# MatthewRalston/kmerdb

Measured on AMD Instinct MI355X. Metric: k-mers counted/sec at k=12, synthetic 150 bp FASTQ, higher is better.
Workload: dtype u64

## Files before the change

### include/kdbhip.h

```cpp
#ifndef KDBHIP_H
#define KDBHIP_H

#include <stddef.h>
#include <stdint.h>

#ifdef __cplusplus
extern "C" {
#endif

#define KDB_ABI_VERSION 6

#define KDB_OK               0
#define KDB_ERR_ARG          1
#define KDB_ERR_HIP          2
#define KDB_ERR_SHORT_READ   3
#define KDB_ERR_BAD_RESIDUE  4
#define KDB_ERR_NOMEM        5
#define KDB_ERR_STATE        6

#define KDB_N_DROP    0
#define KDB_N_EXPAND  1

typedef struct kdb_engine kdb_engine;

// ... 14 lines not shown
#define KDB_SUBMIT_PINNED     1
#define KDB_SUBMIT_CONTINUES  2
int kdb_submit_ex(kdb_engine *e, const uint8_t *bases, size_t nbytes,
                  const uint64_t *read_offsets, size_t nreads, int flags);
int kdb_host_alloc(void **out, size_t nbytes);
int kdb_host_free(void *p);

int kdb_submit_device(kdb_engine *e, void *d_bases, size_t nbytes,
                      const void *d_read_offsets, size_t nreads);

int kdb_submit_device_const(kdb_engine *e, const void *d_bases, size_t nbytes,
                            const void *d_read_offsets, size_t nreads);

int kdb_sync(kdb_engine *e);

int kdb_finish(kdb_engine *e, uint64_t *counts_out, uint64_t *total_kmers, uint64_t *unique_kmers);

int kdb_table_stats(kdb_engine *e, uint64_t *counts_out, uint64_t *sum_out, uint64_t *unique_out);

int kdb_nullomers(kdb_engine *e, int folded, uint64_t *ids_out, uint64_t cap, uint64_t *n_out);

#define KDB_REDUCE_MAX 16
int kdb_reduce(kdb_engine *const *engines, int n, int root);

#define KDB_GRAM_MAX 64
#define KDB_GRAM_BLOCK 4
#define KDB_GRAM_WG_BINS 512
int kdb_gram(int device_id, const void *const *d_vectors, int n, uint64_t nbins,
             uint64_t *sums_out   ,
             uint64_t *gram_out   ,
             double   *kernel_ms_out );

int kdb_fold_file(kdb_engine *e, uint64_t *total_kmers, uint64_t *unique_kmers);
int kdb_fold_file_into(kdb_engine *e, kdb_engine *acc, uint64_t *total_kmers, uint64_t *unique_kmers);
int kdb_finish_folded(kdb_engine *e, uint64_t *counts_out, uint64_t *total_kmers, uint64_t *unique_kmers);

int kdb_table(kdb_engine *e, void **d_table_out, uint64_t *nbins_out);

int kdb_error_counts(kdb_engine *e, uint64_t *n_short_reads, uint64_t *n_bad_residues);

int kdb_create_ids(int k, int canonicalize, int device_id, kdb_engine **out);

int kdb_shred(kdb_engine *e, const uint8_t *seq, size_t nbytes,
              uint64_t *ids_out, uint64_t *pos_out, size_t cap, size_t *n_out);

int kdb_window_ids(kdb_engine *e, const uint8_t *bases, size_t nbytes,
// ... 23 lines not shown
int kdb_gz_read(kdb_gz *g, uint8_t *dst, size_t cap, size_t *n_out);
int kdb_gz_close(kdb_gz *g);

int kdb_write_kdb_rows(const char *path, const uint64_t *counts, uint64_t nbins, uint64_t total_kmers,
                       int compresslevel, int nthreads, uint64_t *nblocks_out);
#define KDB_ENCODER_DEFAULT (-1)
#define KDB_ENCODER_ROWS      0
#define KDB_ENCODER_ZLIB      1
int kdb_write_kdb_rows_ex(const char *path, const uint64_t *counts, uint64_t nbins, uint64_t total_kmers,
                          int compresslevel, int nthreads, int encoder, uint64_t *nblocks_out);
int kdb_format_frequency(uint64_t count, uint64_t total, char *buf, size_t cap);
int kdb_copy_back_and_write_kdb_rows(kdb_engine *e, int folded, uint64_t *counts_out, const char *path, uint64_t total_kmers,
                                     int compresslevel, int nthreads, int encoder, uint64_t *nblocks_out);
int kdb_read_kdb_rows(const char *path, uint64_t nbins, uint64_t *kmer_ids_out, uint64_t *counts_out, double *frequencies_out,
                      int nthreads, uint64_t *nrows_out);

#define KDB_KERNEL_MARK          0
#define KDB_KERNEL_COUNT         1
#define KDB_KERNEL_SCATTER       2
#define KDB_KERNEL_SCATTER_L2    3
#define KDB_KERNEL_PAGE_SORT     4
#define KDB_KERNEL_PAGE_HIST     5
#define KDB_KERNEL_STATS         6
#define KDB_N_KERNELS            7
int         kdb_prof_enable(kdb_engine *e, int on);
int         kdb_prof_reset(kdb_engine *e);
int         kdb_prof_get(kdb_engine *e, int kernel_id, double *total_ms, uint64_t *launches);
const char *kdb_prof_kernel_name(int kernel_id);

int         kdb_hbm_pattern_count(void);
const char *kdb_hbm_pattern_name(int i);
int         kdb_hbm_pattern_probe(int device_id, double *gb_per_s_out, int n_out);
int kdb_set_option(kdb_engine *e, const char *name, int64_t value);
int kdb_get_option(kdb_engine *e, const char *name, int64_t *value);

#ifdef __cplusplus
}
#endif
#endif
```

### kmerdb_amd/_abi.py

```python
import ctypes
import os
import subprocess

_HERE = os.path.dirname(os.path.abspath(__file__))
LIB_PATH = os.environ.get("KDB_LIB") or os.path.join(_HERE, "libkdbhip.so")
CSRC = os.path.join(_HERE, "csrc")
INCLUDE = os.path.join(os.path.dirname(_HERE), "include")

KDB_OK, KDB_ERR_ARG, KDB_ERR_HIP, KDB_ERR_SHORT_READ, KDB_ERR_BAD_RESIDUE, KDB_ERR_NOMEM, KDB_ERR_STATE = range(7)
KDB_N_DROP, KDB_N_EXPAND = 0, 1
KDB_SUBMIT_PINNED, KDB_SUBMIT_CONTINUES = 1, 2
KDB_N_KERNELS = 7
KDB_GRAM_MAX, KDB_GRAM_BLOCK, KDB_GRAM_WG_BINS = 64, 4, 512
ABI_VERSION = 6

_u8p = ctypes.POINTER(ctypes.c_uint8)
_u64p = ctypes.POINTER(ctypes.c_uint64)
_vp = ctypes.c_void_p
SYMBOLS = (
    ("kdb_abi_version", ctypes.c_int, []),
    ("kdb_last_error", ctypes.c_char_p, []),
    ("kdb_device_count", ctypes.c_int, [ctypes.POINTER(ctypes.c_int)]),
    ("kdb_create", ctypes.c_int, [ctypes.c_int, ctypes.c_int, ctypes.c_int, ctypes.c_int, _vp, ctypes.POINTER(_vp)]),
    ("kdb_destroy", ctypes.c_int, [_vp]),
    ("kdb_reset", ctypes.c_int, [_vp]),
    ("kdb_submit", ctypes.c_int, [_vp, _vp, ctypes.c_size_t, _vp, ctypes.c_size_t]),
    ("kdb_submit_pinned", ctypes.c_int, [_vp, _vp, ctypes.c_size_t, _vp, ctypes.c_size_t]),
    ("kdb_submit_ex", ctypes.c_int, [_vp, _vp, ctypes.c_size_t, _vp, ctypes.c_size_t, ctypes.c_int]),
    ("kdb_host_alloc", ctypes.c_int, [ctypes.POINTER(_vp), ctypes.c_size_t]),
    ("kdb_host_free", ctypes.c_int, [_vp]),
    ("kdb_submit_device", ctypes.c_int, [_vp, _vp, ctypes.c_size_t, _vp, ctypes.c_size_t]),
    ("kdb_submit_device_const", ctypes.c_int, [_vp, _vp, ctypes.c_size_t, _vp, ctypes.c_size_t]),
    ("kdb_sync", ctypes.c_int, [_vp]),
    ("kdb_finish", ctypes.c_int, [_vp, _vp, _u64p, _u64p]),
    ("kdb_table_stats", ctypes.c_int, [_vp, _vp, _u64p, _u64p]),
    ("kdb_nullomers", ctypes.c_int, [_vp, ctypes.c_int, _vp, ctypes.c_uint64, _u64p]),
    ("kdb_reduce", ctypes.c_int, [ctypes.POINTER(ctypes.c_void_p), ctypes.c_int, ctypes.c_int]),
    ("kdb_gram", ctypes.c_int, [ctypes.c_int, ctypes.POINTER(ctypes.c_void_p), ctypes.c_int, ctypes.c_uint64, _u64p, _u64p,
                                ctypes.POINTER(ctypes.c_double)]),
    ("kdb_fold_file", ctypes.c_int, [_vp, _u64p, _u64p]),
    ("kdb_fold_file_into", ctypes.c_int, [_vp, _vp, _u64p, _u64p]),
    ("kdb_finish_folded", ctypes.c_int, [_vp, _vp, _u64p, _u64p]),
    ("kdb_create_ids", ctypes.c_int, [ctypes.c_int, ctypes.c_int, ctypes.c_int, ctypes.POINTER(_vp)]),
    ("kdb_table", ctypes.c_int, [_vp, ctypes.POINTER(_vp), _u64p]),
    ("kdb_error_counts", ctypes.c_int, [_vp, _u64p, _u64p]),
    ("kdb_shred", ctypes.c_int, [_vp, _vp, ctypes.c_size_t, _vp, _vp, ctypes.c_size_t, ctypes.POINTER(ctypes.c_size_t)]),
    ("kdb_window_ids", ctypes.c_int, [_vp, _vp, ctypes.c_size_t, _vp, ctypes.c_size_t, _vp]),
    ("kdb_parse_fastq", ctypes.c_int, [_vp, ctypes.c_size_t, ctypes.c_int, _vp, ctypes.c_size_t, _vp, ctypes.c_size_t, _vp,
                                       ctypes.POINTER(ctypes.c_size_t), ctypes.POINTER(ctypes.c_size_t), ctypes.POINTER(ctypes.c_size_t)]),
    ("kdb_parse_fastq_mt", ctypes.c_int, [_vp, ctypes.c_size_t, ctypes.c_int, _vp, ctypes.c_size_t, _vp, ctypes.c_size_t, _vp,
                                          ctypes.POINTER(ctypes.c_size_t), ctypes.POINTER(ctypes.c_size_t), ctypes.POINTER(ctypes.c_size_t), ctypes.c_int]),
    ("kdb_parse_fasta", ctypes.c_int, [_vp, ctypes.c_size_t, _vp, ctypes.c_size_t, _vp, ctypes.c_size_t, _vp,
                                       ctypes.POINTER(ctypes.c_size_t), ctypes.POINTER(ctypes.c_size_t)]),
    ("kdb_parse_fasta_chunk", ctypes.c_int, [_vp, ctypes.c_size_t, ctypes.c_int, ctypes.c_int, _vp, ctypes.c_size_t, _vp, ctypes.c_size_t, _vp,
                                             ctypes.POINTER(ctypes.c_size_t), ctypes.POINTER(ctypes.c_size_t), ctypes.POINTER(ctypes.c_size_t),
                                             ctypes.POINTER(ctypes.c_int)]),
    ("kdb_bgzf_inflate", ctypes.c_int, [_vp, ctypes.c_size_t, _vp, ctypes.c_size_t, ctypes.c_int, ctypes.POINTER(ctypes.c_size_t),
                                        ctypes.POINTER(ctypes.c_size_t)]),
    ("kdb_bgzf_scan", ctypes.c_int, [ctypes.c_char_p, _vp, _vp, ctypes.c_size_t, ctypes.POINTER(ctypes.c_size_t)]),
    ("kdb_gz_open", ctypes.c_int, [ctypes.c_char_p, ctypes.POINTER(_vp)]),
    ("kdb_gz_read", ctypes.c_int, [_vp, _vp, ctypes.c_size_t, ctypes.POINTER(ctypes.c_size_t)]),
    ("kdb_gz_close", ctypes.c_int, [_vp]),
# ... 100 lines not shown
```

### kmerdb_amd/csrc/kdb_engine.hip

```cpp
#include <hip/hip_runtime.h>

#include <cstdarg>
#include <cstddef>
#include <cstdio>
#include <cstdlib>
#include <algorithm>
#include <atomic>
#include <cstring>
#include <string>
#include <thread>
#include <vector>

#include "../../include/kdbhip.h"
#include "kdb_kernels.hip.h"
#include "kdb_hist.hip.h"
#include "kdb_scatter.hip.h"
#include "kdb_scatter_host.hip.h"
#include "kdb_smallk.hip.h"
#include "kdb_probe.hip.h"
#include "kdb_gram.hip.h"
#include "kdb_hostparse.cpp.h"
#include "kdb_kdbwriter.cpp.h"

namespace {

thread_local std::string g_err;

int fail(int code, const char *fmt, ...)
{
    char buf[1024];
    va_list ap;
    va_start(ap, fmt);
    vsnprintf(buf, sizeof buf, fmt, ap);
    va_end(ap);
    g_err = buf;
    return code;
}

#define HIP_TRY(expr)                                                                         \
    do {                                                                                      \
        hipError_t _e = (expr);                                                               \
        if (_e != hipSuccess)                                                                 \
            return fail(KDB_ERR_HIP, "%s failed: %s (%s:%d)", #expr, hipGetErrorString(_e),   \
                        __FILE__, __LINE__);                                                  \
    } while (0)

constexpr int NBUF = 2;
const char *const KERNEL_NAMES[KDB_N_KERNELS] = {
    "lens+mark_reads_kernel", "count_kernel", "scatter_bases_kernel", "scatter_ids_kernel", "pages_sort_kernels", "page_hist_kernel", "stats_kernel"};

struct ProfSpan { hipEvent_t a, b; int kernel; };

void parallel_copy(uint8_t *dst, const uint8_t *src, size_t n, int nthreads)
{
    const size_t min_piece = 4u << 20;
    int t = (int)std::min<size_t>((size_t)std::max(nthreads, 1), std::max<size_t>(n / min_piece, 1));
    if (t <= 1) { if (n) memcpy(dst, src, n); return; }
    std::vector<std::thread> th;
    th.reserve((size_t)t - 1);
    const size_t piece = (n / (size_t)t + 63) & ~(size_t)63;
    for (int i = 1; i < t; i++) {
        const size_t a = std::min(n, piece * (size_t)i), b = std::min(n, piece * (size_t)(i + 1));
        if (b > a) th.emplace_back([=] { memcpy(dst + a, src + a, b - a); });
    }
    memcpy(dst, src, std::min(n, piece));
    for (auto &x : th) x.join();
}

void touch_pages(void *buf, size_t n, int nthreads)
{
    if (n < (64u << 20)) return;
    uint8_t *p = (uint8_t *)buf;
// ... 43 lines not shown
    hipEvent_t ev_acc_done[2] = {nullptr, nullptr};
    hipEvent_t ev_acc_copied = nullptr;
    hipEvent_t ev_pin[2] = {nullptr, nullptr};
    bool pin_used[2] = {false, false};
    int pin_idx = 0;
    bool acc_inflight[2] = {false, false};
    int acc_slot = 0;
    size_t acc_nb = 0, acc_nr = 0;
    bool acc_ready = false;

    int64_t algo = 0;
    int min_len = 0;
    int smallk_old = 0;
    kdb::PagedOptions opt;
    kdb::ScatterState sc;
    int overlap = 0;
    int overlap_hist_cus = 0;
    int overlap_mask_mode = 0;
    bool compute_masked = false;
    hipStream_t s_hist = nullptr;
    kdb::OverlapState ov;
    kdb::TwoLevelPaged tp;
    int64_t oom_fallbacks = 0;

    bool tableless = false;
    uint8_t *sh_seq = nullptr; size_t sh_seq_cap = 0;
    uint64_t *sh_offs = nullptr; size_t sh_offs_cap = 0;
    unsigned long long *sh_ids = nullptr; size_t sh_ids_cap = 0;
    kdb::DevCounters *sh_ctr = nullptr;

    unsigned long long *d_acc_table = nullptr;
    uint64_t folded_files = 0, folded_total = 0;
    uint64_t d2h_bytes = 0;
    uint64_t bytes_in = 0;

    bool prof = false;
    std::vector<ProfSpan> spans;
    std::vector<hipEvent_t> ev_pool;
    double prof_ms[KDB_N_KERNELS] = {0};
    uint64_t prof_n[KDB_N_KERNELS] = {0};
};

namespace {

struct DeviceGuard {
    int prev = -1;
// ... 126 lines not shown
    HIP_TRY(hipExtStreamCreateWithCUMask(&e->s_compute, (uint32_t)ms.size(), ms.data()));
    e->compute_masked = true;
    HIP_TRY(hipExtStreamCreateWithCUMask(&e->s_hist, (uint32_t)mh.size(), mh.data()));
    e->ov.grid = 2u * (uint32_t)(ncu - given);
    return KDB_OK;
}

enum : int { BATCH_HOST_FED = 1, BATCH_CONST_INPUT = 2 };
int grow(void **p, size_t *cap, size_t need_bytes);
int launch_batch(kdb_engine *e, uint8_t *d_bases, size_t nbytes, const uint64_t *d_offs, size_t nreads, int first_is_continuation, int flags);

int flush_accumulated(kdb_engine *e)
{
    if (!e->acc_ready || e->acc_nr == 0) return KDB_OK;
    const int s = e->acc_slot;
    HIP_TRY(hipEventRecord(e->ev_acc_copied, e->s_copy));
    HIP_TRY(hipStreamWaitEvent(e->s_compute, e->ev_acc_copied, 0));
    int rc = launch_batch(e, e->d_acc_bases[s], e->acc_nb, e->d_acc_offs[s], e->acc_nr, 0, BATCH_HOST_FED);
    if (rc != KDB_OK) return rc;
    HIP_TRY(hipEventRecord(e->ev_acc_done[s], e->s_compute));
    e->acc_inflight[s] = true;
    e->acc_slot = s ^ 1;
    e->acc_nb = e->acc_nr = 0;
    return KDB_OK;
}

int launch_batch(kdb_engine *e, uint8_t *d_bases, size_t nbytes, const uint64_t *d_offs, size_t nreads, int first_is_continuation, int flags)
{
    if (nreads == 0) return KDB_OK;
    if (e->tableless) return fail(KDB_ERR_STATE, "this engine was created by kdb_create_ids: it has no count vector");
    const uint64_t ntiles = (nbytes + kdb::TILE_BYTES - 1) / kdb::TILE_BYTES;
    if (ntiles > 0x7FFFFFFFull) return fail(KDB_ERR_ARG, "batch too large: %zu bytes", nbytes);
    bool marked = false;
    auto mark = [&]() {
        ProfScope ps(e, KDB_KERNEL_MARK);
        const unsigned mg = (unsigned)std::min<uint64_t>((nreads + 255) / 256, 4096);
        if (flags & BATCH_CONST_INPUT)
            hipLaunchKernelGGL(kdb::require_uniform_kernel, dim3(1), dim3(1), 0, e->s_compute, e->d_ctr);
        else {
            hipLaunchKernelGGL(kdb::mark_reads_kernel, dim3(mg), dim3(256), 0, e->s_compute, d_bases, d_offs, (uint64_t)nreads,
                               first_is_continuation, e->d_ctr);
            marked = true;
        }
    };
    auto unmark = [&]() {
        if (!marked) return;
// ... 8 lines not shown
        const size_t need = ((nbytes >> kdb::FIRST_REC_SHIFT) + 2) * sizeof(uint32_t);
        if (e->first_rec_cap < need && e->d_first_rec) HIP_TRY(hipStreamSynchronize(e->s_compute));
        int grc = grow((void **)&e->d_first_rec, &e->first_rec_cap, need);
        if (grc == KDB_ERR_NOMEM) no_first_rec = true;
        else if (grc != KDB_OK) return grc;
    }
    {
        ProfScope ps(e, KDB_KERNEL_MARK);
        const dim3 grid((unsigned)((nreads + 255) / 256)), block(256);
        HIP_TRY(hipMemsetAsync(&e->d_ctr->neg_min_len, 0, kdb::PER_BATCH_WORDS * sizeof(unsigned long long), e->s_compute));
        const dim3 lgrid(grid.x < 1024u ? grid.x : 1024u);
        hipLaunchKernelGGL(kdb::lens_kernel, lgrid, block, 0, e->s_compute, d_offs, (uint64_t)nreads, (uint64_t)nbytes,
                           e->min_len > 0 ? e->min_len : e->k, first_is_continuation, e->d_ctr, e->d_first_rec);
    }
    if (nbytes == 0) return KDB_OK;
    if (nreads > 0xFFFFFFF0ull) return fail(KDB_ERR_ARG, "batch of %zu records: at most 2^32 - 16 per submit", nreads);
    e->bytes_in += nbytes;
    const kdb::RecStarts rs{d_offs, e->d_first_rec, (uint32_t)nreads, first_is_continuation ? 1u : 0u};
    int algo = (int)e->algo;
    if (algo == 0 || algo == 3) algo = 2;
    if (no_first_rec && algo == 2) { algo = 1; e->oom_fallbacks++; e->tp.table_is_zero = false; }
    const bool paged2 = algo == 2 && e->k > e->opt.one_level_max_k;
    if (!paged2 || e->n_mode == KDB_N_EXPAND || !e->opt.defer) e->tp.table_is_zero = false;
    if (algo == 2) {
        EngineProf hook(e);
        const bool ex = e->n_mode == KDB_N_EXPAND;
        const kdb::ScBatch batch{d_bases, nbytes, rs, e->k, e->canonical, ex, e->d_table, e->d_ctr};
        int rc;
        if (e->k <= kdb::SMALLK_LDS_MAX_K && !e->smallk_old)
            rc = kdb::smallk_lds_count(e->s_compute, d_bases, nbytes, rs, e->k, e->canonical, ex, e->opt.grid, e->d_table, e->d_ctr, hook);
        else if (e->k <= kdb::SMALLK_MAX) {
            mark();
            rc = kdb::smallk_count(e->s_compute, d_bases, nbytes, e->k, e->canonical, ex, e->d_table, e->d_ctr, hook);
            unmark();
        }
        else if (e->k <= e->opt.one_level_max_k) {
            rc = 3;
            if (e->overlap && e->s_hist && !ex) rc = kdb::scatter_count_overlapped(e->ov, e->opt, e->s_compute, e->s_hist, batch, hook);
            if (rc == 3) {
                { const int jrc = overlap_join(e); if (jrc != KDB_OK) return jrc; }
                rc = kdb::scatter_count(e->sc, e->opt, e->s_compute, batch, hook);
            }
        }
        else {
            const size_t lost = nreads * (size_t)(e->k - 1);
            rc = kdb::twolevel_paged_count(e->tp, e->opt, e->s_compute, batch, nbytes > lost ? nbytes - lost : 0, hook);
        }
        if (rc == 2) { e->oom_fallbacks++; algo = 1; e->tp.table_is_zero = false; }
        else if (rc != 0) return fail(KDB_ERR_HIP, "LDS-histogram path failed: %s", kdb::partition_error());
    }
    if (algo == 1) {
        { const int jrc = overlap_join(e); if (jrc != KDB_OK) return jrc; }
        mark();
        {
            ProfScope ps(e, KDB_KERNEL_COUNT);
            const bool ex = (e->n_mode == KDB_N_EXPAND);
            const dim3 grid((unsigned)ntiles), block(kdb::TPB);
#define KDB_LAUNCH_DIRECT(ID, EX)                                                                              \
    hipLaunchKernelGGL((kdb::count_direct_kernel<ID, EX>), grid, block, 0, e->s_compute, d_bases, (uint64_t)nbytes, \
                       e->k, e->canonical, e->d_table, e->d_ctr)
            if (e->k <= 16) { if (ex) KDB_LAUNCH_DIRECT(uint32_t, true); else KDB_LAUNCH_DIRECT(uint32_t, false); }
            else            { if (ex) KDB_LAUNCH_DIRECT(uint64_t, true); else KDB_LAUNCH_DIRECT(uint64_t, false); }
#undef KDB_LAUNCH_DIRECT
        }
        unmark();
    }
    if (e->n_mode == KDB_N_EXPAND && e->d_worklist) {
        ProfScope ps(e, KDB_KERNEL_COUNT);
        hipLaunchKernelGGL(kdb::expand_worklist_kernel, dim3(1024), dim3(256), 0, e->s_compute, e->d_table, e->d_ctr, e->k, e->canonical);
    }
    if (e->n_mode == KDB_N_DROP) {
        ProfScope ps(e, KDB_KERNEL_MARK);
        hipLaunchKernelGGL(kdb::resolve_suspects_kernel, dim3(4), dim3(256), 0, e->s_compute, (const uint8_t *)d_bases, (uint64_t)nbytes, d_offs, (uint64_t)nreads,
                           e->k, e->d_ctr);
    }
    HIP_TRY(hipGetLastError());
    return KDB_OK;
}

int flush_pending_paged(kdb_engine *e)
{
    if (e->tp.pending == 0) return KDB_OK;
    EngineProf hook(e);
    if (kdb::twolevel_paged_flush(e->tp, e->opt, e->s_compute, e->d_table, e->d_ctr, hook)) return fail(KDB_ERR_HIP, "LDS-histogram path failed: %s", kdb::partition_error());
    return KDB_OK;
}

int check_errors(kdb_engine *e)
{
    kdb::DevCounters c;
    HIP_TRY(hipMemcpy(&c, e->d_ctr, sizeof c, hipMemcpyDeviceToHost));
    if (c.n_short)
// ... 76 lines not shown
    hipLaunchKernelGGL((kdbprobe::pattern<RM, WM, NR, NW>), dim3(512), dim3(512), 0, st, src, sb, dst, db, steps, sink);
}
using namespace kdbprobe;
#define KDB_PROBE(name, RM, WM, NR, NW) {name, probe_launch<RM, WM, NR, NW>, (uint32_t)(NR * (RM == R_PAGES15 ? 1536 : RM ? 1024 : 0)), (uint32_t)(NW * (WM ? 1024 : 0))}
const ProbePattern PROBES[] = {
    KDB_PROBE("stream_read", R_STREAM, W_NONE, 4, 0),
    KDB_PROBE("stream_write", R_NONE, W_STREAM, 0, 4),
    KDB_PROBE("pages_1k_read", R_PAGES, W_NONE, 4, 0),
    KDB_PROBE("lines_64_write", R_NONE, W_LINES_SC1, 0, 2),
    KDB_PROBE("pieces_128_write", R_NONE, W_CHUNK128_SC1, 0, 2),
    KDB_PROBE("scatter_64", R_STREAM, W_LINES_SC1, 1, 2),
    KDB_PROBE("scatter_128", R_STREAM, W_CHUNK128_SC1, 1, 2),
    KDB_PROBE("level1_64", R_STREAM, W_LINES_SC1, 1, 3),
    KDB_PROBE("level1_128", R_STREAM, W_CHUNK128_SC1, 1, 3),
    KDB_PROBE("level2_64", R_PAGES15, W_LINES_SC1, 2, 2),
    KDB_PROBE("level2_128", R_PAGES15, W_CHUNK128_SC1, 2, 2),
};
#undef KDB_PROBE
constexpr int N_PROBES = (int)(sizeof(PROBES) / sizeof(PROBES[0]));
}

namespace {
enum OptBefore { OPT_NOTHING, OPT_FLUSH_PENDING , OPT_SYNC_AND_STREAMS ,
                 OPT_NO_STAGING  };
struct OptRow {
    const char *name;
    int64_t (*get)(kdb_engine *);
    void (*set)(kdb_engine *, int64_t) = nullptr;
    bool boolean = false;
    int64_t lo = INT64_MIN, hi = INT64_MAX;
    OptBefore before = OPT_NOTHING;
    const char *hint = "";
    int64_t multiple_of = 1;
};
#define KDB_OPT_RO(field) [](kdb_engine *e) { return (int64_t)e->field; }
#define KDB_OPT(field) KDB_OPT_RO(field), [](kdb_engine *e, int64_t v) { e->field = (decltype(e->field))v; }
const OptRow OPTIONS[] = {
    {"algo", KDB_OPT(algo), false, 0, 3, OPT_NOTHING, " (0 auto, 1 direct atomics, 2 LDS-histogram paths)"},
    {"min_len", KDB_OPT(min_len), false, 0, 64},
    {"copy_threads", KDB_OPT(copy_threads), false, 1, 64},
    {"smallk_old", KDB_OPT(smallk_old), true},
    {"accum_bytes", KDB_OPT(accum_bytes), false, -1, INT64_MAX, OPT_NO_STAGING, " (-1 auto, 0 off, else bytes)"},
    {"stage_bytes", KDB_OPT(stage_bytes), false, 4096, INT64_MAX, OPT_NO_STAGING, " (>=4096, multiple of 16)", 16},
    {"stage_reads", KDB_OPT(stage_reads), false, 1, INT64_MAX, OPT_NO_STAGING},
    {"overlap", KDB_OPT(overlap), true, 0, 1024, OPT_SYNC_AND_STREAMS},
    {"overlap_hist_cus", KDB_OPT(overlap_hist_cus), false, 0, 1024, OPT_SYNC_AND_STREAMS},
    {"overlap_mask_mode", KDB_OPT(overlap_mask_mode), false, 0, 1024, OPT_SYNC_AND_STREAMS},
    {"sc_grid", KDB_OPT(opt.grid), false, 0, 1024, OPT_NOTHING, " (0..1024)"},
    {"sc_lo_bits", KDB_OPT(opt.lo_bits), false, 0, kdb::SC_LO_BITS_MAX, OPT_FLUSH_PENDING, " (0 = the default of the path, 1..15)"},
    {"sc_contig_pages", KDB_OPT(opt.contig_pages), true},
    {"sc_wide_lines", KDB_OPT(opt.wide_lines), true},
    {"l1_wide_lines", KDB_OPT(opt.l1_wide), true},
    {"l2_wide_lines", KDB_OPT(opt.l2_wide), true},
    {"l1_one_round", KDB_OPT(opt.l1_one_round), true},
    {"l1_compiled_k", KDB_OPT(opt.l1k), true},
    {"one_level_max_k", KDB_OPT(opt.one_level_max_k), false, 12, kdb::SC1_K, OPT_FLUSH_PENDING, " (12 or 13)"},
    {"defer_flush", KDB_OPT(opt.defer), true},
    {"pending_budget", KDB_OPT(opt.budget_bytes), false, 0, INT64_MAX},
    {"reserve_bytes", KDB_OPT(opt.reserve_bytes), false, 0, INT64_MAX},
    {"arena_grow", KDB_OPT(opt.grow), false, 0, 2, OPT_NOTHING, " (0 never, 1 when it pays, 2 whenever the arena has filled up)"},
    {"arena_batches", KDB_OPT(opt.first_batches), false, 1, kdb::PAGED_PENDING_MAX, OPT_NOTHING, " (1..64: the arena's first size, in batches like the first one)"},
    {"k", KDB_OPT_RO(k)},
    {"arena_budget_bytes", [](kdb_engine *e) { return (int64_t)(e->opt.budget_bytes ? e->opt.budget_bytes : e->tp.budget_decided); }},
    {"free_at_sizing", KDB_OPT_RO(tp.free_at_sizing)},
    {"overlap_scatter_grid", KDB_OPT_RO(ov.grid)},
    {"oom_fallbacks", KDB_OPT_RO(oom_fallbacks)},
    {"pending_batches", KDB_OPT_RO(tp.pending)},
    {"d2h_bytes", KDB_OPT_RO(d2h_bytes)},
    {"folded_files", KDB_OPT_RO(folded_files)},
    {"bytes_in", KDB_OPT_RO(bytes_in)},
// ... 127 lines not shown
        if (e->h_bases[b]) (void)hipHostFree(e->h_bases[b]);
        if (e->h_offs[b]) (void)hipHostFree(e->h_offs[b]);
        if (e->d_bases[b]) (void)hipFree(e->d_bases[b]);
        if (e->d_offs[b]) (void)hipFree(e->d_offs[b]);
        if (e->ev_copied[b]) (void)hipEventDestroy(e->ev_copied[b]);
        if (e->ev_done[b]) (void)hipEventDestroy(e->ev_done[b]);
    }
    for (int s2 = 0; s2 < 2; s2++) {
        if (e->d_acc_bases[s2]) (void)hipFree(e->d_acc_bases[s2]);
        if (e->d_acc_offs[s2]) (void)hipFree(e->d_acc_offs[s2]);
        if (e->ev_acc_done[s2]) (void)hipEventDestroy(e->ev_acc_done[s2]);
    }
    if (e->ev_acc_copied) (void)hipEventDestroy(e->ev_acc_copied);
    for (int s2 = 0; s2 < 2; s2++) if (e->ev_pin[s2]) (void)hipEventDestroy(e->ev_pin[s2]);
    if (e->d_worklist) (void)hipFree(e->d_worklist);
    if (e->d_suspects) (void)hipFree(e->d_suspects);
    if (e->d_first_rec) (void)hipFree(e->d_first_rec);
    if (e->sh_suspects) (void)hipFree(e->sh_suspects);
    if (e->sh_seq) (void)hipFree(e->sh_seq);
    if (e->sh_offs) (void)hipFree(e->sh_offs);
    if (e->sh_ids) (void)hipFree(e->sh_ids);
    if (e->sh_ctr) (void)hipFree(e->sh_ctr);
    if (e->d_acc_table) (void)hipFree(e->d_acc_table);
    if (e->d_ctr) (void)hipFree(e->d_ctr);
    if (e->owns_table && e->d_table) (void)hipFree(e->d_table);
    if (e->s_compute) (void)hipStreamDestroy(e->s_compute);
    if (e->s_copy) (void)hipStreamDestroy(e->s_copy);
    delete e;
    return KDB_OK;
}

int kdb_reset(kdb_engine *e)
{
    if (!e) return fail(KDB_ERR_ARG, "engine is NULL");
    DeviceGuard g(e->device);
    e->acc_nb = e->acc_nr = 0;
    kdb::twolevel_paged_drop(e->tp);
    HIP_TRY(hipStreamSynchronize(e->s_copy));
    HIP_TRY(hipStreamSynchronize(e->s_compute));
    if (e->s_hist) { HIP_TRY(hipStreamSynchronize(e->s_hist)); e->ov.last = -1; }
    if (e->nbins) HIP_TRY(hipMemsetAsync(e->d_table, 0, e->nbins * 8ull, e->s_compute));
    if (e->d_acc_table) HIP_TRY(hipMemsetAsync(e->d_acc_table, 0, e->nbins * 8ull, e->s_compute));
    e->folded_files = e->folded_total = 0;
    e->tp.table_is_zero = e->owns_table && !e->table_escaped;
    HIP_TRY(hipMemsetAsync(e->d_ctr, 0, sizeof(kdb::DevCounters), e->s_compute));
    unsigned long long wl[2] = {0, 0}, sus[2] = {0, 0};
    if (e->n_mode == KDB_N_EXPAND) {
        if (!e->d_worklist) HIP_TRY(hipMalloc((void **)&e->d_worklist, e->worklist_cap * sizeof(unsigned long long)));
        wl[0] = (unsigned long long)(uintptr_t)e->d_worklist; wl[1] = (unsigned long long)e->worklist_cap;
        HIP_TRY(hipMemcpyAsync(&e->d_ctr->wl, wl, sizeof wl, hipMemcpyHostToDevice, e->s_compute));
    } else if (!e->tableless) {
        if (!e->d_suspects) HIP_TRY(hipMalloc((void **)&e->d_suspects, e->suspects_cap * sizeof(unsigned long long)));
        sus[0] = (unsigned long long)(uintptr_t)e->d_suspects; sus[1] = (unsigned long long)e->suspects_cap;
        HIP_TRY(hipMemcpyAsync(&e->d_ctr->sus, sus, sizeof sus, hipMemcpyHostToDevice, e->s_compute));
    }
    HIP_TRY(hipStreamSynchronize(e->s_compute));
    return KDB_OK;
}

int kdb_submit_device(kdb_engine *e, void *d_bases, size_t nbytes, const void *d_read_offsets, size_t nreads)
{
    if (!e) return fail(KDB_ERR_ARG, "engine is NULL");
    if (nreads && (!d_bases || !d_read_offsets)) return fail(KDB_ERR_ARG, "NULL device buffer");
    if (((uintptr_t)d_bases & 15u) != 0) return fail(KDB_ERR_ARG, "d_bases must be 16-byte aligned");
    DeviceGuard g(e->device);
// ... 113 lines not shown
}

int kdb_host_alloc(void **out, size_t nbytes)
{
    if (!out) return fail(KDB_ERR_ARG, "out is NULL");
    *out = nullptr;
    hipError_t err = hipHostMalloc(out, nbytes ? nbytes : 1, hipHostMallocDefault);
    if (err != hipSuccess) return fail(KDB_ERR_NOMEM, "hipHostMalloc(%zu) failed: %s", nbytes, hipGetErrorString(err));
    return KDB_OK;
}

int kdb_host_free(void *p)
{
    if (p) HIP_TRY(hipHostFree(p));
    return KDB_OK;
}

int kdb_sync(kdb_engine *e)
{
    if (!e) return fail(KDB_ERR_ARG, "engine is NULL");
    DeviceGuard g(e->device);
    { int rc = flush_accumulated(e); if (rc != KDB_OK) return rc; }
    { int rc = flush_pending_paged(e); if (rc != KDB_OK) return rc; }
    HIP_TRY(hipStreamSynchronize(e->s_copy));
    HIP_TRY(hipStreamSynchronize(e->s_compute));
    if (e->s_hist) { HIP_TRY(hipStreamSynchronize(e->s_hist)); e->ov.last = -1; }
    for (int b = 0; b < NBUF; b++) e->inflight[b] = false;
    e->acc_inflight[0] = e->acc_inflight[1] = false;
    if (e->prof) { int rc = prof_collect(e); if (rc != KDB_OK) return rc; }
#ifdef KDB_SC_PROF
    {
        unsigned long long h[32];
        if (hipMemcpyFromSymbol(h, HIP_SYMBOL(kdb::g_sc_prof), sizeof h) == hipSuccess && (h[8] || h[24])) {
            static const char *names[8] = {"ids", "requests+stage-next+writes", "barrier 1", "flush", "barrier 2", "drain", "flush: word, page turn, line list", "flush: list read, line read, store"};
            static const char *kern[2] = {"scatter_bases_kernel", "scatter_ids_kernel"};
            for (int s2 = 0; s2 < 2; s2++) {
                const unsigned long long *g = h + 16 * s2;
                if (!g[8]) continue;
                unsigned long long tot = 0;
                for (int q = 0; q < 8; q++) tot += g[q];
                fprintf(stderr, "[sc_prof] %s: %llu workgroups; wave-cycles by phase:", kern[s2], g[8]);
                for (int q = 0; q < 8; q++) fprintf(stderr, " %s %.1f%%", names[q], 100.0 * (double)g[q] / (double)tot);
                fprintf(stderr, " | total %.3g wave-cycles\n", (double)tot);
            }
            memset(h, 0, sizeof h);
            (void)hipMemcpyToSymbol(HIP_SYMBOL(kdb::g_sc_prof), h, sizeof h);
// ... 219 lines not shown
        *kernel_ms_out = (double)ms;
    }
    for (uint32_t r = 0; r < nrows; r++) {
        const ulonglong2 *slot = &res[(size_t)r * NSLOT];
        for (int i = 0; i < B; i++) {
            const int vi = rows[r].bi * B + i;
            if (vi >= n) continue;
            if (rows[r].bi == rows[r].bj) { sums_out[2 * vi] = slot[B * B + i].x; sums_out[2 * vi + 1] = slot[B * B + i].y; }
            for (int j = 0; j < B; j++) {
                const int vj = rows[r].bj * B + j;
                if (vj >= n || vj < vi) continue;
                const ulonglong2 v = slot[i * B + j];
                gram_out[2 * ((size_t)vi * n + vj)] = gram_out[2 * ((size_t)vj * n + vi)] = v.x;
                gram_out[2 * ((size_t)vi * n + vj) + 1] = gram_out[2 * ((size_t)vj * n + vi) + 1] = v.y;
            }
        }
    }
    for (int i = 0; i < n; i++)
        if (sums_out[2 * i + 1] != 0)
            return fail(KDB_ERR_ARG, "kdb_gram: the sum of vector %d is 2^64 or more: its products may have wrapped 128 bits", i);
    return KDB_OK;
}

int kdb_reduce(kdb_engine *const *engines, int n, int root)
{
    if (!engines || n < 2 || n > KDB_REDUCE_MAX) return fail(KDB_ERR_ARG, "kdb_reduce: n=%d engines (2..%d)", n, KDB_REDUCE_MAX);
    if (root < 0 || root >= n) return fail(KDB_ERR_ARG, "kdb_reduce: root=%d of %d", root, n);
    for (int j = 0; j < n; j++) {
        kdb_engine *e = engines[j];
        if (!e) return fail(KDB_ERR_ARG, "kdb_reduce: engine %d is NULL", j);
        if (e->tableless) return fail(KDB_ERR_STATE, "kdb_reduce: engine %d was created by kdb_create_ids: it has no count vector", j);
        if (e->k != engines[0]->k) return fail(KDB_ERR_ARG, "kdb_reduce: engine %d counts k=%d, engine 0 k=%d", j, e->k, engines[0]->k);
        if (((uintptr_t)e->d_table & 15u) != 0) return fail(KDB_ERR_ARG, "kdb_reduce: the count vector of engine %d is not 16-byte aligned", j);
        for (int i = 0; i < j; i++)
            if (engines[i] == e || engines[i]->d_table == e->d_table) return fail(KDB_ERR_ARG, "kdb_reduce: engines %d and %d are the same vector", i, j);
    }
    for (int j = 0; j < n; j++) { int rc = kdb_sync(engines[j]); if (rc != KDB_OK) return rc; }
    for (int j = 0; j < n; j++)
        for (int i = 0; i < n; i++) {
            const int dj = engines[j]->device, di = engines[i]->device;
            if (dj == di) continue;
            DeviceGuard g(dj);
            int can = 0;
            HIP_TRY(hipDeviceCanAccessPeer(&can, dj, di));
            if (!can) return fail(KDB_ERR_HIP, "kdb_reduce: device %d cannot access the memory of device %d", dj, di);
            const hipError_t pe = hipDeviceEnablePeerAccess(di, 0);
// ... 450 lines not shown
    if (src) (void)hipFree(src);
    if (dst) (void)hipFree(dst);
    if (sink) (void)hipFree(sink);
    return rc;
}

int kdb_set_option(kdb_engine *e, const char *name, int64_t value)
{
    if (!e || !name) return fail(KDB_ERR_ARG, "NULL argument");
    if (!strcmp(name, "sc_top_bits")) return kdb_set_option(e, "sc_lo_bits", value ? kdb::SC_LO_BITS_MAX : 0);
#ifdef KDB_SC_PROF
    if (!strcmp(name, "sc_ablate")) { int v = (int)value; (void)hipMemcpyToSymbol(HIP_SYMBOL(kdb::g_sc_ablate), &v, sizeof v); return KDB_OK; }
#endif
    const OptRow *row = find_option(name);
    if (!row || !row->set) return fail(KDB_ERR_ARG, "unknown option '%s'", name);
    if (row->before == OPT_NO_STAGING && e->staging_ready) return fail(KDB_ERR_STATE, "staging already allocated");
    if (value < row->lo || value > row->hi || value % row->multiple_of) return fail(KDB_ERR_ARG, "%s=%lld%s", name, (long long)value, row->hint);
    if (row->before == OPT_FLUSH_PENDING || (!strcmp(name, "defer_flush") && !value)) {
        DeviceGuard g(e->device);
        int rc = flush_pending_paged(e);
        if (rc != KDB_OK) return rc;
    }
    if (!strcmp(name, "pending_budget")) e->tp.budget_decided = 0;
    if (row->before != OPT_SYNC_AND_STREAMS) { row->set(e, row->boolean ? (value ? 1 : 0) : value); return KDB_OK; }
    DeviceGuard g(e->device);
    { int rc = kdb_sync(e); if (rc != KDB_OK) return rc; }
    row->set(e, row->boolean ? (value ? 1 : 0) : value);
    return overlap_streams(e);
}

int kdb_get_option(kdb_engine *e, const char *name, int64_t *value)
{
    if (!e || !name || !value) return fail(KDB_ERR_ARG, "NULL argument");
    if (const OptRow *row = find_option(name)) { *value = row->get(e); return KDB_OK; }
    if (!strcmp(name, "free_hbm")) {
        DeviceGuard g(e->device);
        size_t free_b = 0, total_b = 0;
        HIP_TRY(hipMemGetInfo(&free_b, &total_b));
        *value = (int64_t)free_b; return KDB_OK;
    }
    if (!strcmp(name, "arena_used_bound") || !strcmp(name, "arena_worst_case") || !strcmp(name, "arena_cursor")) {
        DeviceGuard g(e->device);
        if (!strcmp(name, "arena_cursor")) {
            uint32_t c = 0;
            HIP_TRY(hipStreamSynchronize(e->s_compute));
            if (e->tp.d_cursor && e->tp.pending) HIP_TRY(hipMemcpy(&c, e->tp.d_cursor, sizeof c, hipMemcpyDeviceToHost));
            *value = (int64_t)c; return KDB_OK;
        }
        kdb::twolevel_paged_poll(e->tp);
        *value = (int64_t)(!strcmp(name, "arena_worst_case") ? e->tp.used2 : e->tp.used2 - e->tp.slack); return KDB_OK;
    }
// ... 20 lines not shown
```

Measured before the change: 709.8 billion.

## Count forward strand only and merge reverse complements in a deferred pass

For canonical counting at small k, the hot counting kernels now run non-canonical into a separate forward table. At sync, a tiled strand-merge kernel folds each k-mer's reverse-complement bin into the canonical bin of the real table. The aim is to drop the per-k-mer reverse-complement and min computation from the hot loop and spread atomics across both strands instead of contending on canonical bins. The cost is an extra table-sized allocation, a memset, and one full merge pass over 4^k bins per sync.

Result: faster. 743.9 billion (median of 6 runs) (+4.8%).

```diff
diff --git a/include/kdbhip.h b/include/kdbhip.h
--- a/include/kdbhip.h
+++ b/include/kdbhip.h
@@ -60,6 +60,8 @@
 
 #define KDB_REDUCE_MAX 16
 int kdb_reduce(kdb_engine *const *engines, int n, int root);
+
+int kdb_strand_merge(int device_id, void *d_fwd, void *d_table, int k);
 
 #define KDB_GRAM_MAX 64
 #define KDB_GRAM_BLOCK 4
@@ -129,7 +131,8 @@
 #define KDB_KERNEL_PAGE_SORT     4
 #define KDB_KERNEL_PAGE_HIST     5
 #define KDB_KERNEL_STATS         6
-#define KDB_N_KERNELS            7
+#define KDB_KERNEL_STRAND_MERGE   7
+#define KDB_N_KERNELS            8
 int         kdb_prof_enable(kdb_engine *e, int on);
 int         kdb_prof_reset(kdb_engine *e);
 int         kdb_prof_get(kdb_engine *e, int kernel_id, double *total_ms, uint64_t *launches);
diff --git a/kmerdb_amd/_abi.py b/kmerdb_amd/_abi.py
--- a/kmerdb_amd/_abi.py
+++ b/kmerdb_amd/_abi.py
@@ -10,7 +10,7 @@
 KDB_OK, KDB_ERR_ARG, KDB_ERR_HIP, KDB_ERR_SHORT_READ, KDB_ERR_BAD_RESIDUE, KDB_ERR_NOMEM, KDB_ERR_STATE = range(7)
 KDB_N_DROP, KDB_N_EXPAND = 0, 1
 KDB_SUBMIT_PINNED, KDB_SUBMIT_CONTINUES = 1, 2
-KDB_N_KERNELS = 7
+KDB_N_KERNELS = 8
 KDB_GRAM_MAX, KDB_GRAM_BLOCK, KDB_GRAM_WG_BINS = 64, 4, 512
 ABI_VERSION = 6
 
@@ -38,6 +38,7 @@
     ("kdb_reduce", ctypes.c_int, [ctypes.POINTER(ctypes.c_void_p), ctypes.c_int, ctypes.c_int]),
     ("kdb_gram", ctypes.c_int, [ctypes.c_int, ctypes.POINTER(ctypes.c_void_p), ctypes.c_int, ctypes.c_uint64, _u64p, _u64p,
                                 ctypes.POINTER(ctypes.c_double)]),
+    ("kdb_strand_merge", ctypes.c_int, [ctypes.c_int, _vp, _vp, ctypes.c_int]),
     ("kdb_fold_file", ctypes.c_int, [_vp, _u64p, _u64p]),
     ("kdb_fold_file_into", ctypes.c_int, [_vp, _vp, _u64p, _u64p]),
     ("kdb_finish_folded", ctypes.c_int, [_vp, _vp, _u64p, _u64p]),
diff --git a/kmerdb_amd/csrc/kdb_engine.hip b/kmerdb_amd/csrc/kdb_engine.hip
--- a/kmerdb_amd/csrc/kdb_engine.hip
+++ b/kmerdb_amd/csrc/kdb_engine.hip
@@ -19,6 +19,7 @@
 #include "kdb_smallk.hip.h"
 #include "kdb_probe.hip.h"
 #include "kdb_gram.hip.h"
+#include "kdb_strands.hip.h"
 #include "kdb_hostparse.cpp.h"
 #include "kdb_kdbwriter.cpp.h"
 
@@ -47,7 +48,7 @@
 
 constexpr int NBUF = 2;
 const char *const KERNEL_NAMES[KDB_N_KERNELS] = {
-    "lens+mark_reads_kernel", "count_kernel", "scatter_bases_kernel", "scatter_ids_kernel", "pages_sort_kernels", "page_hist_kernel", "stats_kernel"};
+    "lens+mark_reads_kernel", "count_kernel", "scatter_bases_kernel", "scatter_ids_kernel", "pages_sort_kernels", "page_hist_kernel", "stats_kernel", "strand_merge_kernel"};
 
 struct ProfSpan { hipEvent_t a, b; int kernel; };
 
@@ -137,6 +138,10 @@
     kdb::OverlapState ov;
     kdb::TwoLevelPaged tp;
     int64_t oom_fallbacks = 0;
+    int strand_merge = 1;
+    int strand_merge_max_k = 12;
+    unsigned long long *d_fwd = nullptr;
+    bool strands_pending = false;
 
     bool tableless = false;
     uint8_t *sh_seq = nullptr; size_t sh_seq_cap = 0;
@@ -309,6 +314,26 @@
     e->acc_inflight[s] = true;
     e->acc_slot = s ^ 1;
     e->acc_nb = e->acc_nr = 0;
+    return KDB_OK;
+}
+
+bool ensure_fwd(kdb_engine *e)
+{
+    if (e->d_fwd) return true;
+    if (hipMalloc((void **)&e->d_fwd, e->nbins * 8ull) != hipSuccess) { (void)hipGetLastError(); e->d_fwd = nullptr; return false; }
+    if (hipMemsetAsync(e->d_fwd, 0, e->nbins * 8ull, e->s_compute) != hipSuccess) { (void)hipGetLastError(); (void)hipFree(e->d_fwd); e->d_fwd = nullptr; return false; }
+    return true;
+}
+
+int merge_strands(kdb_engine *e)
+{
+    if (!e->strands_pending) return KDB_OK;
+    {
+        ProfScope ps(e, KDB_KERNEL_STRAND_MERGE);
+        kdbstrands::strand_merge_launch(e->s_compute, e->d_fwd, e->d_table, e->k);
+    }
+    e->strands_pending = false;
+    HIP_TRY(hipGetLastError());
     return KDB_OK;
 }
 
@@ -363,16 +388,21 @@
     if (no_first_rec && algo == 2) { algo = 1; e->oom_fallbacks++; e->tp.table_is_zero = false; }
     const bool paged2 = algo == 2 && e->k > e->opt.one_level_max_k;
     if (!paged2 || e->n_mode == KDB_N_EXPAND || !e->opt.defer) e->tp.table_is_zero = false;
+    const bool staged = e->canonical && e->strand_merge && algo == 2 && e->k <= std::min((int)e->opt.one_level_max_k, e->strand_merge_max_k) &&
+                        !e->overlap && !e->smallk_old && ensure_fwd(e);
+    const int canonical = staged ? 0 : e->canonical;
+    unsigned long long *const table = staged ? e->d_fwd : e->d_table;
+    if (staged) e->strands_pending = true;
     if (algo == 2) {
         EngineProf hook(e);
         const bool ex = e->n_mode == KDB_N_EXPAND;
-        const kdb::ScBatch batch{d_bases, nbytes, rs, e->k, e->canonical, ex, e->d_table, e->d_ctr};
+        const kdb::ScBatch batch{d_bases, nbytes, rs, e->k, canonical, ex, table, e->d_ctr};
         int rc;
         if (e->k <= kdb::SMALLK_LDS_MAX_K && !e->smallk_old)
-            rc = kdb::smallk_lds_count(e->s_compute, d_bases, nbytes, rs, e->k, e->canonical, ex, e->opt.grid, e->d_table, e->d_ctr, hook);
+            rc = kdb::smallk_lds_count(e->s_compute, d_bases, nbytes, rs, e->k, canonical, ex, e->opt.grid, table, e->d_ctr, hook);
         else if (e->k <= kdb::SMALLK_MAX) {
             mark();
-            rc = kdb::smallk_count(e->s_compute, d_bases, nbytes, e->k, e->canonical, ex, e->d_table, e->d_ctr, hook);
+            rc = kdb::smallk_count(e->s_compute, d_bases, nbytes, e->k, canonical, ex, table, e->d_ctr, hook);
             unmark();
         }
         else if (e->k <= e->opt.one_level_max_k) {
@@ -399,7 +429,7 @@
             const dim3 grid((unsigned)ntiles), block(kdb::TPB);
 #define KDB_LAUNCH_DIRECT(ID, EX)                                                                              \
     hipLaunchKernelGGL((kdb::count_direct_kernel<ID, EX>), grid, block, 0, e->s_compute, d_bases, (uint64_t)nbytes, \
-                       e->k, e->canonical, e->d_table, e->d_ctr)
+                       e->k, canonical, table, e->d_ctr)
             if (e->k <= 16) { if (ex) KDB_LAUNCH_DIRECT(uint32_t, true); else KDB_LAUNCH_DIRECT(uint32_t, false); }
             else            { if (ex) KDB_LAUNCH_DIRECT(uint64_t, true); else KDB_LAUNCH_DIRECT(uint64_t, false); }
 #undef KDB_LAUNCH_DIRECT
@@ -408,7 +438,7 @@
     }
     if (e->n_mode == KDB_N_EXPAND && e->d_worklist) {
         ProfScope ps(e, KDB_KERNEL_COUNT);
-        hipLaunchKernelGGL(kdb::expand_worklist_kernel, dim3(1024), dim3(256), 0, e->s_compute, e->d_table, e->d_ctr, e->k, e->canonical);
+        hipLaunchKernelGGL(kdb::expand_worklist_kernel, dim3(1024), dim3(256), 0, e->s_compute, table, e->d_ctr, e->k, canonical);
     }
     if (e->n_mode == KDB_N_DROP) {
         ProfScope ps(e, KDB_KERNEL_MARK);
@@ -531,7 +561,7 @@
 
 namespace {
 enum OptBefore { OPT_NOTHING, OPT_FLUSH_PENDING , OPT_SYNC_AND_STREAMS ,
-                 OPT_NO_STAGING  };
+                 OPT_SYNC , OPT_NO_STAGING  };
 struct OptRow {
     const char *name;
     int64_t (*get)(kdb_engine *);
@@ -555,6 +585,8 @@
     {"overlap", KDB_OPT(overlap), true, 0, 1024, OPT_SYNC_AND_STREAMS},
     {"overlap_hist_cus", KDB_OPT(overlap_hist_cus), false, 0, 1024, OPT_SYNC_AND_STREAMS},
     {"overlap_mask_mode", KDB_OPT(overlap_mask_mode), false, 0, 1024, OPT_SYNC_AND_STREAMS},
+    {"strand_merge", KDB_OPT(strand_merge), true, 0, 1024, OPT_SYNC},
+    {"strand_merge_max_k", KDB_OPT(strand_merge_max_k), false, 1, 17, OPT_SYNC, " (1..17; never more than one_level_max_k)"},
     {"sc_grid", KDB_OPT(opt.grid), false, 0, 1024, OPT_NOTHING, " (0..1024)"},
     {"sc_lo_bits", KDB_OPT(opt.lo_bits), false, 0, kdb::SC_LO_BITS_MAX, OPT_FLUSH_PENDING, " (0 = the default of the path, 1..15)"},
     {"sc_contig_pages", KDB_OPT(opt.contig_pages), true},
@@ -728,6 +760,7 @@
     if (e->sh_ids) (void)hipFree(e->sh_ids);
     if (e->sh_ctr) (void)hipFree(e->sh_ctr);
     if (e->d_acc_table) (void)hipFree(e->d_acc_table);
+    if (e->d_fwd) (void)hipFree(e->d_fwd);
     if (e->d_ctr) (void)hipFree(e->d_ctr);
     if (e->owns_table && e->d_table) (void)hipFree(e->d_table);
     if (e->s_compute) (void)hipStreamDestroy(e->s_compute);
@@ -747,6 +780,7 @@
     if (e->s_hist) { HIP_TRY(hipStreamSynchronize(e->s_hist)); e->ov.last = -1; }
     if (e->nbins) HIP_TRY(hipMemsetAsync(e->d_table, 0, e->nbins * 8ull, e->s_compute));
     if (e->d_acc_table) HIP_TRY(hipMemsetAsync(e->d_acc_table, 0, e->nbins * 8ull, e->s_compute));
+    if (e->strands_pending) { HIP_TRY(hipMemsetAsync(e->d_fwd, 0, e->nbins * 8ull, e->s_compute)); e->strands_pending = false; }
     e->folded_files = e->folded_total = 0;
     e->tp.table_is_zero = e->owns_table && !e->table_escaped;
     HIP_TRY(hipMemsetAsync(e->d_ctr, 0, sizeof(kdb::DevCounters), e->s_compute));
@@ -906,6 +940,7 @@
     DeviceGuard g(e->device);
     { int rc = flush_accumulated(e); if (rc != KDB_OK) return rc; }
     { int rc = flush_pending_paged(e); if (rc != KDB_OK) return rc; }
+    { int rc = merge_strands(e); if (rc != KDB_OK) return rc; }
     HIP_TRY(hipStreamSynchronize(e->s_copy));
     HIP_TRY(hipStreamSynchronize(e->s_compute));
     if (e->s_hist) { HIP_TRY(hipStreamSynchronize(e->s_hist)); e->ov.last = -1; }
@@ -1171,6 +1206,23 @@
     return KDB_OK;
 }
 
+int kdb_strand_merge(int device_id, void *d_fwd, void *d_table, int k)
+{
+    if (k < 1 || k > 17) return fail(KDB_ERR_ARG, "kdb_strand_merge: k=%d outside 1..17", k);
+    if (!d_fwd || !d_table || d_fwd == d_table) return fail(KDB_ERR_ARG, "kdb_strand_merge: d_fwd and d_table must be two vectors");
+    if ((((uintptr_t)d_fwd | (uintptr_t)d_table) & 7u) != 0) return fail(KDB_ERR_ARG, "kdb_strand_merge: the vectors must be 8-byte aligned");
+    int ndev = 0;
+    HIP_TRY(hipGetDeviceCount(&ndev));
+    if (device_id < 0 || device_id >= ndev) return fail(KDB_ERR_ARG, "device_id=%d but %d device(s) visible", device_id, ndev);
+    DeviceGuard g(device_id);
+    struct Stream { hipStream_t st = nullptr; ~Stream() { if (st) (void)hipStreamDestroy(st); } } s;
+    HIP_TRY(hipStreamCreateWithFlags(&s.st, hipStreamNonBlocking));
+    kdbstrands::strand_merge_launch(s.st, (unsigned long long *)d_fwd, (unsigned long long *)d_table, k);
+    HIP_TRY(hipGetLastError());
+    HIP_TRY(hipStreamSynchronize(s.st));
+    return KDB_OK;
+}
+
 int kdb_reduce(kdb_engine *const *engines, int n, int root)
 {
     if (!engines || n < 2 || n > KDB_REDUCE_MAX) return fail(KDB_ERR_ARG, "kdb_reduce: n=%d engines (2..%d)", n, KDB_REDUCE_MAX);
@@ -1667,11 +1719,11 @@
         if (rc != KDB_OK) return rc;
     }
     if (!strcmp(name, "pending_budget")) e->tp.budget_decided = 0;
-    if (row->before != OPT_SYNC_AND_STREAMS) { row->set(e, row->boolean ? (value ? 1 : 0) : value); return KDB_OK; }
+    if (row->before != OPT_SYNC_AND_STREAMS && row->before != OPT_SYNC) { row->set(e, row->boolean ? (value ? 1 : 0) : value); return KDB_OK; }
     DeviceGuard g(e->device);
     { int rc = kdb_sync(e); if (rc != KDB_OK) return rc; }
     row->set(e, row->boolean ? (value ? 1 : 0) : value);
-    return overlap_streams(e);
+    return row->before == OPT_SYNC ? KDB_OK : overlap_streams(e);
 }
 
 int kdb_get_option(kdb_engine *e, const char *name, int64_t *value)
diff --git a/kmerdb_amd/csrc/kdb_strands.hip.h b/kmerdb_amd/csrc/kdb_strands.hip.h
--- /dev/null
+++ b/kmerdb_amd/csrc/kdb_strands.hip.h
@@ -0,0 +1,97 @@
+#pragma once
+#include <hip/hip_runtime.h>
+#include <stdint.h>
+
+namespace kdbstrands {
+
+constexpr int STRAND_DIRECT_MAX_K = 8;
+constexpr int TPB = 256;
+constexpr int TILE = 64;
+constexpr int ROWS = TILE / (TPB / 64);
+
+__host__ __device__ __forceinline__ uint64_t rc_id(uint64_t x, int k)
+{
+    uint64_t v = ~x;
+    v = ((v >> 2) & 0x3333333333333333ull) | ((v & 0x3333333333333333ull) << 2);
+    v = ((v >> 4) & 0x0F0F0F0F0F0F0F0Full) | ((v & 0x0F0F0F0F0F0F0F0Full) << 4);
+    v = ((v >> 8) & 0x00FF00FF00FF00FFull) | ((v & 0x00FF00FF00FF00FFull) << 8);
+    v = ((v >> 16) & 0x0000FFFF0000FFFFull) | ((v & 0x0000FFFF0000FFFFull) << 16);
+    v = (v >> 32) | (v << 32);
+    return v >> (64 - 2 * k);
+}
+
+__global__ __launch_bounds__(TPB) void
+strand_merge_direct_kernel(unsigned long long *__restrict__ F, unsigned long long *__restrict__ table, int k)
+{
+    const uint64_t nbins = 1ull << (2 * k);
+    for (uint64_t i = (uint64_t)blockIdx.x * TPB + threadIdx.x; i < nbins; i += (uint64_t)gridDim.x * TPB) {
+        const uint64_t r = rc_id(i, k);
+        if (i > r) continue;
+        unsigned long long s = F[i];
+        if (i < r) { s += F[r]; F[r] = 0; }
+        F[i] = 0;
+        if (s) table[i] += s;
+    }
+}
+
+__global__ __launch_bounds__(TPB) void
+strand_merge_kernel(unsigned long long *__restrict__ F, unsigned long long *__restrict__ table, int k)
+{
+    __shared__ unsigned long long T[2][TILE * TILE];
+    const int km = k - 6;
+    const uint32_t M0 = blockIdx.x, M1 = (uint32_t)rc_id(M0, km);
+    if (M1 < M0) return;
+    const bool self = M1 == M0;
+    const int ntiles = self ? 1 : 2;
+    const uint64_t a_stride = 1ull << (2 * (k - 3));
+    const uint32_t lane = threadIdx.x & 63u, wave = threadIdx.x >> 6;
+    const uint64_t base[2] = {(uint64_t)M0 * TILE + lane, (uint64_t)M1 * TILE + lane};
+
+    const uint64_t row_step = (uint64_t)(TPB / 64) * a_stride;
+    for (int t = 0; t < ntiles; t++) {
+        unsigned long long *p = F + (uint64_t)wave * a_stride + base[t];
+        unsigned long long v[ROWS];
+#pragma unroll
+        for (int j = 0; j < ROWS; j++) v[j] = p[(uint64_t)j * row_step];
+#pragma unroll
+        for (int j = 0; j < ROWS; j++) {
+            const uint32_t A = wave + (uint32_t)j * (TPB / 64);
+            T[t][A * TILE + (lane ^ A)] = v[j];
+            p[(uint64_t)j * row_step] = 0;
+        }
+    }
+    __syncthreads();
+
+    const uint32_t rcB = (uint32_t)rc_id(lane, 3);
+    for (int t = 0; t < ntiles; t++) {
+        const int o = self ? 0 : 1 - t;
+        const bool m_less = t == 0 && !self;
+        unsigned long long s[ROWS], old[ROWS];
+#pragma unroll
+        for (int j = 0; j < ROWS; j++) {
+            const uint32_t A = wave + (uint32_t)j * (TPB / 64);
+            const bool less = A < rcB || (A == rcB && m_less);
+            const bool same = A == rcB && self;
+            s[j] = 0;
+            if (less || same) s[j] = T[t][A * TILE + (lane ^ A)];
+            if (less) { const uint32_t rcA = (uint32_t)rc_id(A, 3); s[j] += T[o][rcB * TILE + (rcA ^ rcB)]; }
+        }
+        unsigned long long *q = table + (uint64_t)wave * a_stride + base[t];
+#pragma unroll
+        for (int j = 0; j < ROWS; j++) if (s[j]) old[j] = q[(uint64_t)j * row_step];
+#pragma unroll
+        for (int j = 0; j < ROWS; j++) if (s[j]) q[(uint64_t)j * row_step] = old[j] + s[j];
+    }
+}
+
+inline void strand_merge_launch(hipStream_t st, unsigned long long *F, unsigned long long *table, int k)
+{
+    if (k <= STRAND_DIRECT_MAX_K) {
+        const uint64_t nbins = 1ull << (2 * k);
+        hipLaunchKernelGGL(strand_merge_direct_kernel, dim3((unsigned)((nbins + TPB - 1) / TPB)), dim3(TPB), 0, st, F, table, k);
+    } else {
+        hipLaunchKernelGGL(strand_merge_kernel, dim3(1u << (2 * (k - 6))), dim3(TPB), 0, st, F, table, k);
+    }
+}
+
+}
```
